# filthyrake/telescope_cam_detection

Hardware: AMD Instinct MI355X
Metric: frames_per_sec (higher is better)
Workload: dtype f16x3; 1 GPU; RT-DETR-R50 640x640 bs=8/GPU, uint8 BGR frames resident in HBM -> [8,300,6] detections in HBM; synthetic seeded weights; global_batch=8, parallelism=camera-shard x1, streams_per_gpu=1, batches_in_flight_per_gpu=1, hip_graph=True

## Files before the change

telescope_cam_detection_amd/csrc/common.h:

```cpp
#pragma once
#include <hip/hip_runtime.h>
#include <stdint.h>
#include <string.h>

#include <stdexcept>
#include <string>
#include <tuple>
#include <type_traits>
#include <utility>
#include <vector>

namespace rtd {

enum DType : int { BF16 = 0, F32 = 1, U8 = 2, I32 = 3, F16X2 = 4 };
constexpr int SPLIT_GROUP = 32;
enum Act : int { ACT_NONE = 0, ACT_RELU = 1, ACT_SILU = 2, ACT_GELU = 3 };
enum ResMode : int { RES_NONE = 0, RES_PRE = 1, RES_POST = 2 };

inline size_t dtype_size(int dt) { return dt == BF16 ? 2 : (dt == U8 ? 1 : 4); }

typedef __bf16 bf16;
typedef __bf16 bf16x8 __attribute__((ext_vector_type(8)));
typedef __bf16 bf16x4 __attribute__((ext_vector_type(4)));
typedef _Float16 sp16;
// ... 125 lines not shown
  const void* pf = nullptr;
  size_t pf_bytes = 0;
};
void launch_conv(const ConvArgs& a, hipStream_t s);
bool conv_dual_supported(const ConvArgs& a);
bool conv_next_supported(const ConvArgs& a);
int conv_kpad(int K);
int conv_kpad_split(int K);
bool conv_split_supported(const ConvArgs& a);
int conv_npad(int N);
bool conv_avg_supported(const ConvArgs& a);
bool conv_sx_batch_fits(const ConvArgs& a);
bool conv_pool_supported(const ConvArgs& a, const Tensor& pooled);
size_t conv_pool_side_bytes(const ConvArgs& a);
void launch_conv_pool(const ConvArgs& a, const Tensor& pooled, void* side, hipStream_t s);
size_t conv_split_slab_bytes(const ConvArgs& a);

void launch_layernorm(const Tensor& x, const Tensor* res, const float* g, const float* b, const Tensor& y,
                      float eps, hipStream_t s);
void launch_add(const Tensor& a, const Tensor& b, const Tensor& y, hipStream_t s);
void launch_maxpool3x3s2(const Tensor& x, const Tensor& y, hipStream_t s);
void launch_upsample2x(const Tensor& x, const Tensor& y, hipStream_t s);
void launch_avgpool2(const Tensor& x, const Tensor& y, hipStream_t s);
void launch_attention(const Tensor& qk, const Tensor& v, const Tensor& o, int heads, hipStream_t s);
void launch_set_rows(const Tensor& y, const int32_t* rows, int nrows, int rows_per_image, const float* vec,
                     hipStream_t s);
void launch_rowmax(const Tensor& x, float* out, hipStream_t s);
void launch_topk(const float* keys, int B, int N, int K, int32_t* idx, float* vals, hipStream_t s);
void launch_gather_rows(const Tensor& src, const int32_t* idx, int rows_per_image, const Tensor& dst, hipStream_t s);
void launch_ref_init(const Tensor& boxdelta, const float* anchors, const int32_t* idx, int S, float* ref_unact8,
// ... 105 lines not shown
__device__ __forceinline__ f32x16 mfma_pair32(const sp16x8& a, const sp16x8& b, const f32x16& c) { return __builtin_amdgcn_mfma_f32_32x32x16_f16(a, b, c, 0, 0, 0); }
__device__ __forceinline__ void split_load8(const sp16* base, long long pix_off, int c, float (&v)[8]) {
  const sp16* q = base + split_off(pix_off, c);
  const sp16x8 h = *(const sp16x8*)q, l = *(const sp16x8*)(q + SPLIT_GROUP);
#pragma unroll
  for (int k = 0; k < 8; ++k) v[k] = (float)h[k] + (float)l[k];
}
__device__ __forceinline__ void split_store8(sp16* base, long long pix_off, int c, const float (&v)[8]) {
  sp16* q = base + split_off(pix_off, c);
  sp16x8 h, l;
#pragma unroll
  for (int k = 0; k < 8; ++k) { sp16 a, b; split2(v[k], a, b); h[k] = a; l[k] = b; }
  *(sp16x8*)q = h;
  *(sp16x8*)(q + SPLIT_GROUP) = l;
}
__device__ __forceinline__ float rows4_max(float v) {
  const auto a = __builtin_amdgcn_permlane16_swap(__float_as_uint(v), __float_as_uint(v), false, false);
  const float t = fmaxf(__uint_as_float(a[0]), __uint_as_float(a[1]));
  const auto b = __builtin_amdgcn_permlane32_swap(__float_as_uint(t), __float_as_uint(t), false, false);
  return fmaxf(__uint_as_float(b[0]), __uint_as_float(b[1]));
}
__device__ __forceinline__ float rows4_sum(float v) {
  const auto a = __builtin_amdgcn_permlane16_swap(__float_as_uint(v), __float_as_uint(v), false, false);
  const float t = __uint_as_float(a[0]) + __uint_as_float(a[1]);
  const auto b = __builtin_amdgcn_permlane32_swap(__float_as_uint(t), __float_as_uint(t), false, false);
  return __uint_as_float(b[0]) + __uint_as_float(b[1]);
}
#define RTD_DPP_ROW_REDUCE(OP)                                                           \
  v = OP(v, __builtin_bit_cast(float, __builtin_amdgcn_update_dpp(0, __builtin_bit_cast(int, v), 0xB1, 0xf, 0xf, false)));   \
  v = OP(v, __builtin_bit_cast(float, __builtin_amdgcn_update_dpp(0, __builtin_bit_cast(int, v), 0x4E, 0xf, 0xf, false)));   \
// ... 23 lines not shown
```

telescope_cam_detection_amd/csrc/conv_igemm.hip:

```cpp
#include <stdlib.h>
#include <string.h>

#include <algorithm>

#include "common.h"

namespace rtd {

struct ConvK {
  const void* x;
  const void* w;
  const float* bias;
  const void* res;
  void* y;
  int M, H, W, Cin;
  long long ldx, x_bstride;
  int OH, OW, OHW;
  int N, Kreal, Kpad;
  int KH, KW, stride, pad;
  long long ldy, y_bstride, ldr, r_bstride;
  int act, res_mode, y_f32, res_f32;
  int ntn;
  const void* pf;
  unsigned pf_bytes;
// ... 1085 lines not shown
  if (four) rtd_launch((conv_igemm_ws_kernel<T, 4>), dim3((unsigned)(mt * ntn)), dim3(512), 0, s, g);
  else rtd_launch((conv_igemm_ws_kernel<T, 2>), dim3((unsigned)(mt * ntn)), dim3(512), 0, s, g);
  return true;
}


struct PoolOut {
  sp16* y;
  long long ldy, bstride;
  int OH, OW;
  unsigned y_bytes;
  sp16* side_row;
  sp16* side_col;
  unsigned row_bytes, col_bytes;
};
template <int COG, bool POOL = false>
__global__ __launch_bounds__(512, 2) void conv3x3_reg_split_kernel(const ConvK a, unsigned x_bytes, unsigned y_bytes, int tiles_x, int tiles_y, int ntiles,
                                                                   const PoolOut po) {
  static_assert(!POOL || COG == 2, "the pooled form is stem.2's (32 -> 64 channels)");
  constexpr int NW = 8, NT_ = 512, WPG = NW / COG, RPW = 8 / WPG;
  constexpr int TH = 8, TW = 32, PW = TW + 2, PH = TH + 2, NPIX = PW * PH;
  constexpr int ROWB = 128, CPP = 8, PPI = 8;
  constexpr int NINSTR = (NPIX + PPI - 1) / PPI;
  constexpr int PBUF = NINSTR * 1024;
  constexpr int ROWO = 128 + 16;
  constexpr int WROW = 9 * 64 * 2 + 16;
  static_assert(32 * COG * WROW <= 2 * PBUF, "the filter is staged through the two patch buffers");
  __shared__ __attribute__((aligned(16))) char patch[2 * PBUF];
  __shared__ __attribute__((aligned(16))) char stage[NW][32 * ROWO];

  const int tid = threadIdx.x, lane = tid & 63;
  const int wv = __builtin_amdgcn_readfirstlane(tid >> 6);
  const int grp = wv / WPG, wq = wv % WPG;
  const int nbase = grp * 32;
  const int h = lane >> 5;

  sp16x8 wf[9][4];
  {
    const sp16* wg = (const sp16*)a.w;
    constexpr int CPR = 9 * 64 / 8;
    for (int e = tid; e < 32 * COG * CPR; e += NT_) {
      const int row = e / CPR, ch = e - row * CPR;
      *(sp16x8*)(patch + row * WROW + ch * 16) = *(const sp16x8*)(wg + (size_t)row * a.Kpad + ch * 8);
    }
    __syncthreads();
#pragma unroll
    for (int tap = 0; tap < 9; ++tap)
#pragma unroll
      for (int kc = 0; kc < 4; ++kc)
        wf[tap][kc] = *(const sp16x8*)(patch + (nbase + (lane & 31)) * WROW + (tap * 64 + kc * 16 + 8 * h) * 2);
    __syncthreads();
  }

  const __amdgpu_buffer_rsrc_t rx = __builtin_amdgcn_make_buffer_rsrc((void*)a.x, 0, x_bytes, 0x00020000);
  const __amdgpu_buffer_rsrc_t ry = __builtin_amdgcn_make_buffer_rsrc(POOL ? (void*)po.y : (void*)a.y, 0, POOL ? po.y_bytes : y_bytes, 0x00020000);
  const __amdgpu_buffer_rsrc_t rsr = __builtin_amdgcn_make_buffer_rsrc((void*)(POOL ? po.side_row : (sp16*)a.y), 0, POOL ? po.row_bytes : 0u, 0x00020000);
  const __amdgpu_buffer_rsrc_t rsc = __builtin_amdgcn_make_buffer_rsrc((void*)(POOL ? po.side_col : (sp16*)a.y), 0, POOL ? po.col_bytes : 0u, 0x00020000);
  auto swz = [](int pi) { return (pi >> 1) & 7; };
  auto issue_patch = [&](int tile, int buf) {
    const int tx = tile % tiles_x;
    const int t2 = tile / tiles_x;
    const int ty = t2 % tiles_y;
    const int b = t2 / tiles_y;
    const int x0 = tx * TW, y0 = ty * TH;
    for (int j = wv; j < NINSTR; j += NW) {
      const int pi = j * PPI + lane / CPP;
      const int py = pi / PW, px = pi - py * PW;
      const int iy = y0 - 1 + py, ix = x0 - 1 + px;
      const bool ok = pi < NPIX && (unsigned)iy < (unsigned)a.H && (unsigned)ix < (unsigned)a.W;
      const int src_chunk = (lane % CPP) ^ swz(pi);
      const unsigned vo = ok ? (unsigned)(((long long)b * a.x_bstride + ((long long)iy * a.W + ix) * a.ldx) * 2 + src_chunk * 16) : 0x80000000u;
      __builtin_amdgcn_raw_ptr_buffer_load_lds(rx, (lds_ptr_t)(patch + buf * PBUF + j * 1024), 16, vo, 0, 0, 0);
    }
  };

  int tile = blockIdx.x;
  if (tile < ntiles) issue_patch(tile, 0);
  for (int it = 0; tile < ntiles; tile += gridDim.x, ++it) {
    const int buf = it & 1;
    if (it == 0) asm volatile("s_waitcnt vmcnt(0)" ::: "memory");
    else if (RPW == 1) asm volatile("s_waitcnt vmcnt(4)" ::: "memory");
    else asm volatile("s_waitcnt vmcnt(8)" ::: "memory");
    __syncthreads();
    if (tile + (int)gridDim.x < ntiles) issue_patch(tile + gridDim.x, buf ^ 1);
    const int tx = tile % tiles_x;
    const int t2 = tile / tiles_x;
    const int ty = t2 % tiles_y;
    const int b = t2 / tiles_y;
    const int x0 = tx * TW, y0 = ty * TH;
    const char* pbuf = patch + buf * PBUF;

    float vm[16];
#pragma unroll
    for (int e = 0; e < 16; ++e) vm[e] = 0.f;
#pragma unroll 1
    for (int rr_ = 0; rr_ < RPW; ++rr_) {
      const int r = wq * RPW + rr_;
      f32x16 acc;
#pragma unroll
      for (int e = 0; e < 16; ++e) acc[e] = 0.f;
      sp16x8 xf[2][4];
      auto read_tap = [&](sp16x8 (&dst)[4], int tap) {
        const int kh = tap / 3, kw = tap - kh * 3;
        const int pi = (r + kh) * PW + kw + (lane & 31);
// ... 794 lines not shown
  k.pf_bytes = (o.prefetch && a.pf && a.pf_bytes < (1ull << 31)) ? (unsigned)a.pf_bytes : 0u;
  const long long x_bytes = ((long long)(x.n - 1) * x.bstride + ((long long)x.h * x.w - 1) * x.ld + x.c) * 4;
  const long long w_bytes = (long long)a.Npad * a.Kpad * 2;
  RTD_CHECK(x_bytes < (1ll << 31) && x2_bytes < (1ll << 31) && w_bytes < (1ll << 31), 1, "conv (f16x3): operand larger than a buffer descriptor (2 GiB)");
  g.splitk = 1; g.x_bytes = (unsigned)x_bytes; g.w_bytes = (unsigned)w_bytes; g.x2_bytes = (unsigned)x2_bytes;
  if (dispatch_sx(k, a, x_bytes, x2_bytes, s)) { HIP_CHECK(hipGetLastError()); return; }
  RTD_CHECK(a.next_y.p == nullptr, 1, "conv (f16x3): a fused following conv exists in the streaming kernel only");
  RTD_CHECK(a.avg_y.p == nullptr, 1, "conv (f16x3): the fused vd-shortcut average exists in the streaming kernel only (the plan must fall back to the avg-pool launch)");
  if (o.conv_reg && a.KH == 3 && a.KW == 3 && a.stride == 1 && a.pad == 1 && !dual && a.res_mode == RES_NONE && x.c == 32 && (y.c == 32 || y.c == 64) &&
      y.dt == F16X2) {
    const long long y_bytes = ((long long)(y.n - 1) * y.bstride + ((long long)y.h * y.w - 1) * y.ld + y.c) * 4;
    const int tiles_x = (x.w + 31) / 32, tiles_y = (x.h + 7) / 8;
    const long long ntiles = (long long)x.n * tiles_x * tiles_y;
    if (tiles_x * tiles_y >= 32 && ntiles < (1ll << 30) && y_bytes < (1ll << 31)) {
      const unsigned gx = (unsigned)std::min<long long>(ntiles, 256);
      if (y.c == 32) rtd_launch((conv3x3_reg_split_kernel<1>), dim3(gx), dim3(512), 0, s, k, (unsigned)x_bytes, (unsigned)y_bytes, tiles_x, tiles_y, (int)ntiles, PoolOut{});
      else rtd_launch((conv3x3_reg_split_kernel<2>), dim3(gx), dim3(512), 0, s, k, (unsigned)x_bytes, (unsigned)y_bytes, tiles_x, tiles_y, (int)ntiles, PoolOut{});
      HIP_CHECK(hipGetLastError());
      return;
    }
  }
  if ((o.conv_reg & 2) && a.KH == 3 && a.KW == 3 && a.stride == 1 && a.pad == 1 && !dual && a.res_mode == RES_NONE && x.c == 64 && y.c == 64 && y.dt == F16X2) {
    const long long y_bytes = ((long long)(y.n - 1) * y.bstride + ((long long)y.h * y.w - 1) * y.ld + y.c) * 4;
    const int tiles_x = (x.w + 15) / 16, tiles_y = (x.h + 7) / 8;
    const long long ntiles = (long long)x.n * tiles_x * tiles_y;
    if (tiles_x * tiles_y >= 128 && ntiles < (1ll << 30) && y_bytes < (1ll << 31)) {
      const unsigned gx = (unsigned)std::min<long long>(ntiles, 256);
      rtd_launch(conv3x3_reg_split64_kernel, dim3(gx), dim3(512), 0, s, k, (unsigned)x_bytes, (unsigned)y_bytes, tiles_x, tiles_y, (int)ntiles);
      HIP_CHECK(hipGetLastError());
      return;
    }
  }
// ... 117 lines not shown
  k.KH = 3; k.KW = 3; k.stride = 1; k.pad = 1;
  k.ldy = 0; k.y_bstride = 0; k.ldr = 0; k.r_bstride = 0; k.res_f32 = 0;
  k.act = a.act; k.res_mode = RES_NONE; k.y_f32 = 0; k.split = 1; k.y_split = 1; k.res_split = 0;
  k.x2 = nullptr; k.ldx2 = 0; k.x2_bstride = 0; k.k2_start = 0; k.ntn = 1; k.reg_epi = 1; k.prefer256 = 0; k.pf = nullptr; k.pf_bytes = 0; k.x_up2 = 0;
  k.next_w = nullptr; k.next_bias = nullptr; k.next_y = nullptr; k.next_ldy = 0; k.next_y_bstride = 0; k.next_kpad = 0; k.next_act = 0;
  const long long x_bytes = ((long long)(x.n - 1) * x.bstride + ((long long)x.h * x.w - 1) * x.ld + x.c) * 4;
  const long long p_bytes = ((long long)(pooled.n - 1) * pooled.bstride + ((long long)pooled.h * pooled.w - 1) * pooled.ld + pooled.c) * 4;
  const int tiles_x = (x.w + 31) / 32, tiles_y = (x.h + 7) / 8;
  const long long ntiles = (long long)x.n * tiles_x * tiles_y;
  RTD_CHECK(x_bytes < (1ll << 31) && p_bytes < (1ll << 31) && ntiles * 8192 < (1ll << 31), 1, "conv + max-pool: operand larger than a buffer descriptor");
  PoolOut po;
  po.y = (sp16*)pooled.p; po.ldy = pooled.ld; po.bstride = pooled.bstride; po.OH = pooled.h; po.OW = pooled.w; po.y_bytes = (unsigned)p_bytes;
  po.side_row = (sp16*)side; po.row_bytes = (unsigned)(ntiles * 8192);
  po.side_col = (sp16*)((char*)side + ntiles * 8192); po.col_bytes = (unsigned)(ntiles * 1024);
  const unsigned gx = (unsigned)std::min<long long>(ntiles, 256);
  rtd_launch((conv3x3_reg_split_kernel<2, true>), dim3(gx), dim3(512), 0, s, k, (unsigned)x_bytes, 0u, tiles_x, tiles_y, (int)ntiles, po);
  HIP_CHECK(hipGetLastError());
  const long long items = ntiles * 19 * (64 / 8);
  rtd_launch(k_pool_fixup, dim3((unsigned)((items + 255) / 256)), dim3(256), 0, s, po, tiles_x, tiles_y, (int)ntiles, 64);
  HIP_CHECK(hipGetLastError());
}

void launch_conv(const ConvArgs& a, hipStream_t s) {
  const Tensor& x = a.x;
  const Tensor& y = a.y;
  if (x.dt == F16X2) { launch_conv_split(a, s); return; }
  const ConvOpts& o = opts_of(a);
  RTD_CHECK(x.dt == BF16 || x.dt == F32, 1, "conv: input dtype");
  RTD_CHECK(y.dt == BF16 || y.dt == F32 || (y.dt == F16X2 && x.dt == F32), 1, "conv: output dtype");
  if (y.dt == F16X2) RTD_CHECK(y.c % SPLIT_GROUP == 0 && y.ld % SPLIT_GROUP == 0 && a.res_mode == RES_NONE && !a.x2.p && !a.next_y.p && ((uintptr_t)y.p & 15) == 0, 1,
                                "conv: fp32 -> F16X2 output needs 32-channel groups and no residual / second input");
  const int epc = x.dt == BF16 ? 8 : 4;
  const int up = a.x_up2 ? 2 : 1;
  if (a.x_up2) RTD_CHECK(a.KH == 1 && a.KW == 1 && a.stride == 1 && a.pad == 0 && a.x2.p, 1, "conv: x_up2 needs a 1x1 conv with a second input");
// ... 73 lines not shown
```

telescope_cam_detection_amd/csrc/engine.hip:

```cpp
#include "engine_internal.h"

using namespace rtd;
using namespace rtd_eng;

namespace rtd {
__thread GraphBuild* t_graph_build = nullptr;
__thread long long t_launches = 0;
}

void launch_force_idx(int32_t* dst, const int32_t* src, const int32_t* flag, int n, hipStream_t s);

namespace rtd_eng {
thread_local std::string g_create_error;
PlanOpts g_opts;
}

namespace rtd_eng {

void parse_blob(rtd_engine* e) {
  const char* b = e->blob.data();
  const size_t n = e->blob.size();
  RTD_CHECK(n >= 12 && memcmp(b, "RTDW", 4) == 0, RTD_E_WEIGHTS, "weight blob: bad magic");
  uint32_t ver, count;
  memcpy(&ver, b + 4, 4);
// ... 479 lines not shown
  Tensor encoder(Flow& F);
  bool dec_fused() const { return e->opts.dec_fused && c.d_model == 256 && c.dec_heads == 8 && c.dec_ffn <= 1024 && c.num_classes <= 512 && c.n_levels == 3 && c.n_points == 4; }
  Queries select_queries(Flow& F, const Tensor& mem);
  Decoded decoder(Flow& F, const Tensor& mem, const Queries& q);
  Tensor decoder_fused(Flow& F, const Queries& q, const Tensor& vall, float* ref8, float* ref_unact8);
  Tensor decoder_by_op(const Queries& q, const Tensor& vall, const Tensor& ref8t, float* ref_unact8);
  void post_process(const Decoded& d);
};

void Builder::stem(Flow& F) {
  const int H = c.input_h, W = c.input_w;
  Tensor x = act(SP ? F32 : P, n, H, W, 8, "input");
  plan->input = x;
  const int eh = c.embedding_size / 2;
  const int h = down2(H), w = down2(W);
  Tensor s0 = act(P, n, h, w, eh);
  plan->stem_fused = SP && e->opts.stem_fused_split && eh == 32;
  if (plan->stem_fused) {
    const uint8_t** table = (const uint8_t**)alloc((size_t)c.max_batch * sizeof(void*));
    plan->frame_table = table;
    if (!dry) {
      DevWeight w0 = get_weight(e, {{"backbone.stem.0", 9 * 8}}, P, eh);
      const void* wp = w0.w; const float* bp = w0.bias; const int kp = w0.Kpad; const int n = this->n;
      push("backbone.stem.0", "conv_igemm", 2.0 * n * h * w * eh * 27.0, (double)n * H * W * 3 + tbytes(s0),
           [table, n, H, W, wp, kp, bp, s0](hipStream_t st) { launch_stem0_u8(table, n, H, W, wp, kp, bp, s0, ACT_RELU, st); });
    }
  } else {
    conv("backbone.stem.0", x, s0, {.k = 3, .stride = 2, .pad = 1, .act = ACT_RELU, .real_cin = 3});
  }
  Tensor s1 = act(P, n, h, w, eh);
  conv("backbone.stem.1", s0, s1, {.k = 3, .pad = 1, .act = ACT_RELU});
  const Tensor s2v = mk(nullptr, P, n, h, w, c.embedding_size);
  const int ph = down2(h), pw = down2(w);
  const ConvSpec stem2{.k = 3, .pad = 1, .act = ACT_RELU};
  const long long pool_tiles = (long long)n * ((w + 31) / 32) * ((h + 7) / 8);
  const bool fuse = SP && e->opts.stem_pool_fuse && conv_pool_supported(probe(s1, s2v, stem2), probe_shape(mk(nullptr, P, n, ph, pw, c.embedding_size), 1)) &&
                    pool_tiles * 8192 < (1ll << 31);
  F.h = ph; F.w = pw;
  if (fuse) {
    F.cur = act(P, n, ph, pw, c.embedding_size, "stem");
    ConvArgs a;
    a.x = s1; a.y = s2v;
    a.KH = a.KW = 3; a.stride = 1; a.pad = 1; a.act = ACT_RELU; a.opts = &e->conv_opts;
    const DevWeight w2 = get_weight(e, {{"backbone.stem.2", 9 * s1.c}}, P, c.embedding_size, dry);
    a.w = w2.w; a.bias = w2.bias; a.Kpad = w2.Kpad; a.Npad = w2.Npad;
    void* side = alloc(conv_pool_side_bytes(a));
// ... 1105 lines not shown
```

telescope_cam_detection_amd/csrc/engine_internal.h:

```cpp
#pragma once
#include <math.h>
#include <string.h>

#include <chrono>
#include <functional>
#include <map>
#include <memory>
#include <mutex>
#include <string>
#include <vector>

#include "../../include/rtdetr_mi355.h"
#include "../../include/rtdetr_mi355_test.h"
#include "common.h"

namespace rtd_eng {
using namespace rtd;

struct PlanOpts {
  int sc_fold = 1;
  int c1_fuse = 1;
  int attn_split = 3;
  int up_fold = 1;
  int arena_reuse = 1;
  int stem_fused_split = 1;
  int aifi_pair = 1;
  int post_fused = 1;
  int dead_out = 1;
  int avg_fuse = 1;
  int stem_pool_fuse = 1;
  int sel_fused = 1;
  int dec_fused = 1;
  int side_stream = 7;
};

struct HostTensor {
  const float* data = nullptr;
  std::vector<int64_t> shape;
  int64_t numel() const {
    int64_t n = 1;
    for (auto d : shape) n *= d;
    return n;
  }
};
// ... 144 lines not shown
```

telescope_cam_detection_amd/csrc/ops.hip:

```cpp
#include <float.h>

#include <algorithm>

#include "common.h"

namespace rtd {

template <typename T> __device__ __forceinline__ float ldf(const T* p) { return (float)(*p); }
template <typename T> __device__ __forceinline__ void stf(T* p, float v) { *p = (T)v; }

__device__ __forceinline__ float wave_sum(float v) { return wave_sum64(v); }

static inline unsigned blocks_for(int64_t n, int per_block) { return (unsigned)((n + per_block - 1) / per_block); }

#define DISPATCH_T(dt, ...)                     \
  do {                                          \
    if ((dt) == BF16) { typedef bf16 T; __VA_ARGS__; } \
    else { typedef float T; __VA_ARGS__; }      \
  } while (0)

template <typename T>
__global__ void k_f32_to(const float* __restrict__ src, T* __restrict__ dst, int64_t n) {
  int64_t i = (int64_t)blockIdx.x * blockDim.x + threadIdx.x;
  if (i < n) dst[i] = (T)src[i];
// ... 1289 lines not shown
  __shared__ __attribute__((aligned(16))) char stage[4][32 * ROWO];
  const int tid = threadIdx.x, lane = tid & 63, wv = tid >> 6, h = lane >> 5;
  int t = blockIdx.x;
  const int tx = t % tiles_x; t /= tiles_x;
  const int ty = t % tiles_y;
  const int b = t / tiles_y;
  const int x0 = tx * TW, y0 = ty * TH;
  const uint8_t* __restrict__ f = table[b];
  const long long fbytes = (long long)H * W * 3;
  const bool aligned4 = (((uintptr_t)f) & 3) == 0;
  for (int e = tid; e < PR * NDW; e += 256) {
    const int r = e / NDW, d = e - r * NDW;
    const int iy = 2 * y0 - 1 + r;
    const long long g0 = ((long long)iy * W + (2 * x0 - 1)) * 3;
    const long long a0 = (g0 & ~3ll) + 4ll * d;
    unsigned dw = 0;
    const bool row_ok = (unsigned)iy < (unsigned)H;
    if (row_ok) {
      if (aligned4 && a0 >= 0 && a0 + 4 <= fbytes) dw = *(const unsigned*)(f + a0);
      else {
#pragma unroll
        for (int q = 0; q < 4; ++q)
          if (a0 + q >= 0 && a0 + q < fbytes) dw |= (unsigned)f[a0 + q] << (8 * q);
      }
    }
#pragma unroll
    for (int q = 0; q < 4; ++q) {
      const int el = (int)(a0 + q - g0);
      if (el < 0 || el >= PC * 3) continue;
      const int ix = 2 * x0 - 1 + el / 3;
      const float v = (row_ok && (unsigned)ix < (unsigned)W) ? (float)((dw >> (8 * q)) & 0xffu) : 0.f;
      const float vn = v / 255.0f;
      const E hi = (E)vn;
      patch[r * ROWE + el] = hi;
      if (SPLIT) patch_lo[r * ROWE + el] = (E)(vn - (float)hi);
    }
  }
  for (int e = tid; e < PR * (ROWE - PC * 3); e += 256) {
    const int r = e / (ROWE - PC * 3), i = e - r * (ROWE - PC * 3);
    patch[r * ROWE + PC * 3 + i] = (E)0.f;
    if (SPLIT) patch_lo[r * ROWE + PC * 3 + i] = (E)0.f;
  }
  Ex8 wf[2], wfl[2];
  int doff[2][4];
#pragma unroll
  for (int s = 0; s < 2; ++s) {
#pragma unroll
    for (int j = 0; j < 8; ++j) {
      const int k = 16 * s + 8 * h + j;
      const int kh = k / 10, e = k - kh * 10;
      const int kw = e / 3, cb = e - kw * 3;
      const int kr = (kh * 3 + kw) * 8 + (2 - cb);
      const bool real = k < 30 && e < 9;
      if (SPLIT) {
        const size_t pos = (size_t)(lane & 31) * Kpad + ((kr >> 5) << 6) + (kr & 31);
        wf[s][j] = real ? wq[pos] : (E)0.f;
        wfl[s][j] = real ? wq[pos + 32] : (E)0.f;
      } else {
        wf[s][j] = real ? wq[(size_t)(lane & 31) * Kpad + kr] : (E)0.f;
      }
    }
#pragma unroll
    for (int j = 0; j < 4; ++j) {
      const int k = 16 * s + 8 * h + 2 * j;
      const int kh = k / 10, e = k - kh * 10;
      doff[s][j] = k < 30 ? kh * ROWE + e : 0;
    }
  }
  __syncthreads();
#pragma unroll 1
  for (int rr = 0; rr < 2; ++rr) {
    const int r = wv * 2 + rr;
    const int eoff = (2 * r) * ROWE + (2 * (lane & 31)) * 3;
    const E* base = patch + eoff;
    f32x16_s acc;
#pragma unroll
    for (int e = 0; e < 16; ++e) acc[e] = 0.f;
#pragma unroll
    for (int s = 0; s < 2; ++s) {
      typedef unsigned u4_s __attribute__((ext_vector_type(4)));
      unsigned xd[4];
#pragma unroll
      for (int j = 0; j < 4; ++j) xd[j] = *(const unsigned*)(base + doff[s][j]);
      const u4_s xv = {xd[0], xd[1], xd[2], xd[3]};
      if constexpr (SPLIT) acc = mfma_pair32(wf[s], __builtin_bit_cast(Ex8, xv), acc);
      else acc = __builtin_amdgcn_mfma_f32_32x32x16_bf16(wf[s], __builtin_bit_cast(Ex8, xv), acc, 0, 0, 0);
      if constexpr (SPLIT) {
        unsigned xl[4];
#pragma unroll
        for (int j = 0; j < 4; ++j) xl[j] = *(const unsigned*)(patch_lo + eoff + doff[s][j]);
        const u4_s xlv = {xl[0], xl[1], xl[2], xl[3]};
        acc = mfma_pair32(wf[s], __builtin_bit_cast(Ex8, xlv), acc);
        acc = mfma_pair32(wfl[s], __builtin_bit_cast(Ex8, xv), acc);
      }
    }
    const int oy = y0 + r;
    char* sw_ = stage[wv];
#pragma unroll
    for (int q = 0; q < 4; ++q) {
      const f32x4_s bv = *(const f32x4_s*)(bias + 8 * q + 4 * h);
      Ex4 o, ol;
#pragma unroll
      for (int e = 0; e < 4; ++e) {
        float v = acc[4 * q + e] + bv[e];
        if (act == ACT_RELU) v = fmaxf(v, 0.f);
        else if (act == ACT_SILU) v = v / (1.f + __expf(-v));
        if constexpr (SPLIT) { sp16 hh, ll; split2(v, hh, ll); o[e] = hh; ol[e] = ll; }
        else o[e] = (E)v;
      }
      *(Ex4*)(sw_ + (lane & 31) * ROWO + (8 * q + 4 * h) * 2) = o;
// ... 69 lines not shown
```

telescope_cam_detection_amd/csrc/testapi.hip:

```cpp
#include "engine_internal.h"

using namespace rtd;
using namespace rtd_eng;

extern "C" {

int rtd_debug_tensor(rtd_handle h, const char* name, float* out, int64_t capacity, int64_t shape[4]) {
  return guarded(h, [&] {
    RTD_CHECK(name && shape && h->last_n > 0, RTD_E_STATE, "no forward has run");
    Plan* p = h->plans[h->last_n].get();
    auto it = p->named.find(name);
    RTD_CHECK(it != p->named.end(), RTD_E_INVALID, std::string("unknown debug tensor ") + name);
    const Tensor& t = it->second;
    if (p->stem_fused && strcmp(name, "input") == 0 && out) {
      HIP_CHECK(hipSetDevice(h->cfg.device));
      launch_preprocess_identity(h->last_fa, h->cfg.input_h, h->cfg.input_w, p->input, p->scale_wh, h->stream);
    }
    shape[0] = t.n; shape[1] = t.h; shape[2] = t.w; shape[3] = t.c;
    const int64_t numel = t.pixels() * t.c;
    if (!out) return;
    RTD_CHECK(capacity >= numel, RTD_E_INVALID, "debug tensor: output capacity too small");
    RTD_CHECK(t.bstride == (int64_t)t.h * t.w * t.ld, RTD_E_INVALID, "debug tensor: non-dense batch stride");
    HIP_CHECK(hipSetDevice(h->cfg.device));
    const size_t es = dtype_size(t.dt);
// ... 147 lines not shown
  for (int i = 0; i < 16; ++i) s += acc[i][0] + acc[i][3];
  if (s == 123.456f) sink[0] = s;
  if (lane == 0) { const int w = blockIdx.x * 4 + (tid >> 6); out[2 * w] = c1 - c0; out[2 * w + 1] = r1 - r0; }
}
static int g_bench_rewarm = 0;
int rtd_debug_option(const char* name, int value) {
  if (!name) return RTD_E_INVALID;
  if (strcmp(name, "reset") == 0) {
    g_opts = PlanOpts();
    g_profile_twice = 0; g_bench_rewarm = 0;
    conv_opts_template() = ConvOpts();
    return RTD_OK;
  }
  const struct { const char* n; int* p; } plan_opts[] = {
      {"dec_fused", &g_opts.dec_fused}, {"side_stream", &g_opts.side_stream}, {"sel_fused", &g_opts.sel_fused},
      {"stem_fused_split", &g_opts.stem_fused_split}, {"stem_pool_fuse", &g_opts.stem_pool_fuse}, {"avg_fuse", &g_opts.avg_fuse}, {"dead_out", &g_opts.dead_out}, {"post_fused", &g_opts.post_fused}, {"aifi_pair", &g_opts.aifi_pair}, {"sc_fold", &g_opts.sc_fold}, {"arena_reuse", &g_opts.arena_reuse},
      {"up_fold", &g_opts.up_fold}, {"attn_split", &g_opts.attn_split}, {"c1_fuse", &g_opts.c1_fuse},
      {"profile_twice", &g_profile_twice}, {"bench_rewarm", &g_bench_rewarm},
  };
  for (const auto& t : plan_opts)
    if (strcmp(name, t.n) == 0) { *t.p = value; return RTD_OK; }
  if (conv_set_option(name, value)) return RTD_OK;
  return RTD_E_INVALID;
}

struct DevFilter {
  float* wpad = nullptr; void* w = nullptr; float* bias = nullptr;
  int Kpad = 0, Npad = 0;
  void release() { if (w != wpad) (void)hipFree(w); (void)hipFree(wpad); (void)hipFree(bias); }
};
static DevFilter dev_filter(int dtype, const void* w_f32, const float* bias, int N, int K) {
// ... 302 lines not shown
```

Measured before the change: 1838 frames/s.

## Fuse stem.0 uint8 conv into stem.1 conv kernel via on-chip recompute

```diff
diff --git a/telescope_cam_detection_amd/csrc/common.h b/telescope_cam_detection_amd/csrc/common.h
--- a/telescope_cam_detection_amd/csrc/common.h
+++ b/telescope_cam_detection_amd/csrc/common.h
@@ -163,6 +163,10 @@
 bool conv_pool_supported(const ConvArgs& a, const Tensor& pooled);
 size_t conv_pool_side_bytes(const ConvArgs& a);
 void launch_conv_pool(const ConvArgs& a, const Tensor& pooled, void* side, hipStream_t s);
+bool stem01_u8_supported(const ConvArgs& a);
+bool stem01_u8_batch_fits(const ConvArgs& a);
+void launch_stem01_u8(const uint8_t* const* table_dev, int n, int H, int W, const void* w0, int Kpad0, const float* bias0, const ConvArgs& a,
+                      hipStream_t s);
 size_t conv_split_slab_bytes(const ConvArgs& a);
 
 void launch_layernorm(const Tensor& x, const Tensor* res, const float* g, const float* b, const Tensor& y,
@@ -298,6 +302,81 @@
   *(sp16x8*)q = h;
   *(sp16x8*)(q + SPLIT_GROUP) = l;
 }
+__device__ __forceinline__ unsigned stem_u8_fetch(const uint8_t* __restrict__ f, long long fbytes, bool aligned4, bool row_ok, long long a0) {
+  unsigned dw = 0;
+  if (row_ok) {
+    if (aligned4 && a0 >= 0 && a0 + 4 <= fbytes) dw = *(const unsigned*)(f + a0);
+    else {
+#pragma unroll
+      for (int q = 0; q < 4; ++q)
+        if (a0 + q >= 0 && a0 + q < fbytes) dw |= (unsigned)f[a0 + q] << (8 * q);
+    }
+  }
+  return dw;
+}
+__device__ __forceinline__ void stem_u8_put(unsigned dw, long long a0, long long g0, bool row_ok, int xbase, int W, int nel, sp16* __restrict__ hi_row,
+                                            sp16* __restrict__ lo_row) {
+#pragma unroll
+  for (int q = 0; q < 4; ++q) {
+    const int el = (int)(a0 + q - g0);
+    if (el < 0 || el >= nel) continue;
+    const int ix = xbase + el / 3;
+    const float v = (row_ok && (unsigned)ix < (unsigned)W) ? (float)((dw >> (8 * q)) & 0xffu) : 0.f;
+    const float vn = v / 255.0f;
+    const sp16 hi = (sp16)vn;
+    hi_row[el] = hi;
+    lo_row[el] = (sp16)(vn - (float)hi);
+  }
+}
+struct Stem0Frags {
+  sp16x8 wh[2], wl[2];
+  int doff[2][4];
+};
+__device__ __forceinline__ Stem0Frags stem0_u8_frags(const sp16* __restrict__ wq, int Kpad, int lane, int rowe) {
+  Stem0Frags fr;
+  const int h = lane >> 5;
+#pragma unroll
+  for (int s = 0; s < 2; ++s) {
+#pragma unroll
+    for (int j = 0; j < 8; ++j) {
+      const int k = 16 * s + 8 * h + j;
+      const int kh = k / 10, e = k - kh * 10;
+      const int kw = e / 3, cb = e - kw * 3;
+      const int kr = (kh * 3 + kw) * 8 + (2 - cb);
+      const bool real = k < 30 && e < 9;
+      const size_t pos = (size_t)(lane & 31) * Kpad + ((kr >> 5) << 6) + (kr & 31);
+      fr.wh[s][j] = real ? wq[pos] : (sp16)0.f;
+      fr.wl[s][j] = real ? wq[pos + 32] : (sp16)0.f;
+    }
+#pragma unroll
+    for (int j = 0; j < 4; ++j) {
+      const int k = 16 * s + 8 * h + 2 * j;
+      const int kh = k / 10, e = k - kh * 10;
+      fr.doff[s][j] = k < 30 ? kh * rowe + e : 0;
+    }
+  }
+  return fr;
+}
+__device__ __forceinline__ f32x16 stem0_u8_mfma(const Stem0Frags& fr, const sp16* hi, const sp16* lo) {
+  typedef unsigned u4_s __attribute__((ext_vector_type(4)));
+  f32x16 acc;
+#pragma unroll
+  for (int e = 0; e < 16; ++e) acc[e] = 0.f;
+#pragma unroll
+  for (int s = 0; s < 2; ++s) {
+    unsigned xd[4], xl[4];
+#pragma unroll
+    for (int j = 0; j < 4; ++j) xd[j] = *(const unsigned*)(hi + fr.doff[s][j]);
+    const u4_s xv = {xd[0], xd[1], xd[2], xd[3]};
+    acc = mfma_pair32(fr.wh[s], __builtin_bit_cast(sp16x8, xv), acc);
+#pragma unroll
+    for (int j = 0; j < 4; ++j) xl[j] = *(const unsigned*)(lo + fr.doff[s][j]);
+    const u4_s xlv = {xl[0], xl[1], xl[2], xl[3]};
+    acc = mfma_pair32(fr.wh[s], __builtin_bit_cast(sp16x8, xlv), acc);
+    acc = mfma_pair32(fr.wl[s], __builtin_bit_cast(sp16x8, xv), acc);
+  }
+  return acc;
+}
 __device__ __forceinline__ float rows4_max(float v) {
   const auto a = __builtin_amdgcn_permlane16_swap(__float_as_uint(v), __float_as_uint(v), false, false);
   const float t = fmaxf(__uint_as_float(a[0]), __uint_as_float(a[1]));
diff --git a/telescope_cam_detection_amd/csrc/conv_igemm.hip b/telescope_cam_detection_amd/csrc/conv_igemm.hip
--- a/telescope_cam_detection_amd/csrc/conv_igemm.hip
+++ b/telescope_cam_detection_amd/csrc/conv_igemm.hip
@@ -1123,10 +1123,18 @@
   sp16* side_col;
   unsigned row_bytes, col_bytes;
 };
-template <int COG, bool POOL = false>
+struct Stem0In {
+  const uint8_t* const* table;
+  int H, W;
+  const sp16* w;
+  int Kpad;
+  const float* bias;
+};
+template <int COG, bool POOL = false, bool U8 = false>
 __global__ __launch_bounds__(512, 2) void conv3x3_reg_split_kernel(const ConvK a, unsigned x_bytes, unsigned y_bytes, int tiles_x, int tiles_y, int ntiles,
-                                                                   const PoolOut po) {
+                                                                   const PoolOut po, const Stem0In s0) {
   static_assert(!POOL || COG == 2, "the pooled form is stem.2's (32 -> 64 channels)");
+  static_assert(!U8 || (COG == 1 && !POOL), "the uint8 form is stem.1's (32 -> 32 channels)");
   constexpr int NW = 8, NT_ = 512, WPG = NW / COG, RPW = 8 / WPG;
   constexpr int TH = 8, TW = 32, PW = TW + 2, PH = TH + 2, NPIX = PW * PH;
   constexpr int ROWB = 128, CPP = 8, PPI = 8;
@@ -1134,9 +1142,22 @@
   constexpr int PBUF = NINSTR * 1024;
   constexpr int ROWO = 128 + 16;
   constexpr int WROW = 9 * 64 * 2 + 16;
-  static_assert(32 * COG * WROW <= 2 * PBUF, "the filter is staged through the two patch buffers");
-  __shared__ __attribute__((aligned(16))) char patch[2 * PBUF];
+  constexpr int NBUF = U8 ? 1 : 2;
+  static_assert(U8 || 32 * COG * WROW <= NBUF * PBUF, "the filter is staged through the patch buffers");
+  __shared__ __attribute__((aligned(16))) char patch_s[NBUF * PBUF];
   __shared__ __attribute__((aligned(16))) char stage[NW][32 * ROWO];
+  constexpr int UR = 2 * PH + 1, UC = 2 * PW + 1, UROW = 212, UNDW = (UC * 3 + 3 + 3) / 4, UPT = (UR * UNDW + NT_ - 1) / NT_;
+  static_assert(UROW % 2 == 0 && UROW >= 6 * (PW - 1) + 10, "a pixel's 10-element filter row stays inside its patch row");
+  __shared__ __attribute__((aligned(16))) sp16 u8hi_s[U8 ? UR * UROW : 8];
+  __shared__ __attribute__((aligned(16))) sp16 u8lo_s[U8 ? UR * UROW : 8];
+  __shared__ __attribute__((aligned(16))) Stem0Frags fr0_s[U8 ? 64 : 1];
+  Stem0Frags* const fr0p = fr0_s;
+  constexpr int RELOAD = 2;
+  __shared__ __attribute__((aligned(16))) char wlds_s[U8 ? 32 * WROW : 16];
+  char* const wbuf = U8 ? wlds_s : patch_s;
+  char* const patch = patch_s;
+  sp16* const u8hi = u8hi_s;
+  sp16* const u8lo = u8lo_s;
 
   const int tid = threadIdx.x, lane = tid & 63;
   const int wv = __builtin_amdgcn_readfirstlane(tid >> 6);
@@ -1150,14 +1171,14 @@
     constexpr int CPR = 9 * 64 / 8;
     for (int e = tid; e < 32 * COG * CPR; e += NT_) {
       const int row = e / CPR, ch = e - row * CPR;
-      *(sp16x8*)(patch + row * WROW + ch * 16) = *(const sp16x8*)(wg + (size_t)row * a.Kpad + ch * 8);
+      *(sp16x8*)(wbuf + row * WROW + ch * 16) = *(const sp16x8*)(wg + (size_t)row * a.Kpad + ch * 8);
     }
     __syncthreads();
 #pragma unroll
     for (int tap = 0; tap < 9; ++tap)
 #pragma unroll
       for (int kc = 0; kc < 4; ++kc)
-        wf[tap][kc] = *(const sp16x8*)(patch + (nbase + (lane & 31)) * WROW + (tap * 64 + kc * 16 + 8 * h) * 2);
+        wf[tap][kc] = *(const sp16x8*)(wbuf + (nbase + (lane & 31)) * WROW + (tap * 64 + kc * 16 + 8 * h) * 2);
     __syncthreads();
   }
 
@@ -1183,20 +1204,98 @@
     }
   };
 
+  const long long fbytes = (long long)s0.H * s0.W * 3;
+  auto u8_item = [&](int tile, int i, const uint8_t*& f, int& r, long long& g0, long long& a0, bool& row_ok, int& xbase) {
+    const int tx = tile % tiles_x;
+    const int t2 = tile / tiles_x;
+    const int ty = t2 % tiles_y;
+    f = s0.table[t2 / tiles_y];
+    const int e = tid + i * NT_;
+    r = e / UNDW;
+    const int iy = 2 * (ty * TH) - 3 + r;
+    xbase = 2 * (tx * TW) - 3;
+    g0 = ((long long)iy * s0.W + xbase) * 3;
+    a0 = (g0 & ~3ll) + 4ll * (e - r * UNDW);
+    row_ok = (unsigned)iy < (unsigned)s0.H;
+    return e < UR * UNDW;
+  };
+  auto u8_fetch = [&](int tile, unsigned (&dw)[UPT]) {
+#pragma unroll
+    for (int i = 0; i < UPT; ++i) {
+      const uint8_t* f; int r, xbase; long long g0, a0; bool row_ok;
+      dw[i] = u8_item(tile, i, f, r, g0, a0, row_ok, xbase) ? stem_u8_fetch(f, fbytes, (((uintptr_t)f) & 3) == 0, row_ok, a0) : 0u;
+    }
+  };
+  auto u8_put = [&](int tile, const unsigned (&dw)[UPT]) {
+#pragma unroll
+    for (int i = 0; i < UPT; ++i) {
+      const uint8_t* f; int r, xbase; long long g0, a0; bool row_ok;
+      if (u8_item(tile, i, f, r, g0, a0, row_ok, xbase)) stem_u8_put(dw[i], a0, g0, row_ok, xbase, s0.W, UC * 3, u8hi + r * UROW, u8lo + r * UROW);
+    }
+  };
+  unsigned udw[UPT];
+
   int tile = blockIdx.x;
-  if (tile < ntiles) issue_patch(tile, 0);
+  if constexpr (U8) {
+    if (tile < ntiles) u8_fetch(tile, udw);
+    if (wv == 0) fr0p[lane] = stem0_u8_frags(s0.w, s0.Kpad, lane, UROW);
+    for (int e = tid; e < UR * (UROW - UC * 3); e += NT_) {
+      const int r = e / (UROW - UC * 3), i = e - r * (UROW - UC * 3);
+      u8hi[r * UROW + UC * 3 + i] = (sp16)0.f;
+      u8lo[r * UROW + UC * 3 + i] = (sp16)0.f;
+    }
+  } else {
+    if (tile < ntiles) issue_patch(tile, 0);
+  }
   for (int it = 0; tile < ntiles; tile += gridDim.x, ++it) {
-    const int buf = it & 1;
-    if (it == 0) asm volatile("s_waitcnt vmcnt(0)" ::: "memory");
-    else if (RPW == 1) asm volatile("s_waitcnt vmcnt(4)" ::: "memory");
-    else asm volatile("s_waitcnt vmcnt(8)" ::: "memory");
-    __syncthreads();
-    if (tile + (int)gridDim.x < ntiles) issue_patch(tile + gridDim.x, buf ^ 1);
+    const int buf = U8 ? 0 : (it & 1);
     const int tx = tile % tiles_x;
     const int t2 = tile / tiles_x;
     const int ty = t2 % tiles_y;
     const int b = t2 / tiles_y;
     const int x0 = tx * TW, y0 = ty * TH;
+    if constexpr (U8) {
+      u8_put(tile, udw);
+      __syncthreads();
+      if (tile + (int)gridDim.x < ntiles) u8_fetch(tile + gridDim.x, udw);
+      const Stem0Frags fr0 = fr0p[lane];
+      for (int g = wv; g * 32 < NPIX; g += NW) {
+        const int pi = g * 32 + (lane & 31), pic = pi < NPIX ? pi : NPIX - 1;
+        const int py = pic / PW, px = pic - py * PW;
+        const int eoff = 2 * py * UROW + 6 * px;
+        const f32x16 acc = stem0_u8_mfma(fr0, u8hi + eoff, u8lo + eoff);
+        const bool in_map = (unsigned)(y0 - 1 + py) < (unsigned)a.H && (unsigned)(x0 - 1 + px) < (unsigned)a.W;
+        char* prow = patch + pic * ROWB;
+        const int sw = swz(pic);
+#pragma unroll
+        for (int q = 0; q < 4; ++q) {
+          const f32x4 bv = *(const f32x4*)(s0.bias + 8 * q + 4 * h);
+          sp16x4 oh, ol;
+#pragma unroll
+          for (int e = 0; e < 4; ++e) {
+            sp16 hi, lo;
+            split2(in_map ? fmaxf(acc[4 * q + e] + bv[e], 0.f) : 0.f, hi, lo);
+            oh[e] = hi; ol[e] = lo;
+          }
+          if (pi < NPIX) {
+            *(sp16x4*)(prow + ((q ^ sw) << 4) + 8 * h) = oh;
+            *(sp16x4*)(prow + (((4 + q) ^ sw) << 4) + 8 * h) = ol;
+          }
+        }
+      }
+      __syncthreads();
+#pragma unroll
+      for (int tap = 9 - RELOAD; tap < 9; ++tap)
+#pragma unroll
+        for (int kc = 0; kc < 4; ++kc)
+          wf[tap][kc] = *(const sp16x8*)(wbuf + (nbase + (lane & 31)) * WROW + (tap * 64 + kc * 16 + 8 * h) * 2);
+    } else {
+      if (it == 0) asm volatile("s_waitcnt vmcnt(0)" ::: "memory");
+      else if (RPW == 1) asm volatile("s_waitcnt vmcnt(4)" ::: "memory");
+      else asm volatile("s_waitcnt vmcnt(8)" ::: "memory");
+      __syncthreads();
+      if (tile + (int)gridDim.x < ntiles) issue_patch(tile + gridDim.x, buf ^ 1);
+    }
     const char* pbuf = patch + buf * PBUF;
 
     float vm[16];
@@ -2021,8 +2120,8 @@
     const long long ntiles = (long long)x.n * tiles_x * tiles_y;
     if (tiles_x * tiles_y >= 32 && ntiles < (1ll << 30) && y_bytes < (1ll << 31)) {
       const unsigned gx = (unsigned)std::min<long long>(ntiles, 256);
-      if (y.c == 32) rtd_launch((conv3x3_reg_split_kernel<1>), dim3(gx), dim3(512), 0, s, k, (unsigned)x_bytes, (unsigned)y_bytes, tiles_x, tiles_y, (int)ntiles, PoolOut{});
-      else rtd_launch((conv3x3_reg_split_kernel<2>), dim3(gx), dim3(512), 0, s, k, (unsigned)x_bytes, (unsigned)y_bytes, tiles_x, tiles_y, (int)ntiles, PoolOut{});
+      if (y.c == 32) rtd_launch((conv3x3_reg_split_kernel<1>), dim3(gx), dim3(512), 0, s, k, (unsigned)x_bytes, (unsigned)y_bytes, tiles_x, tiles_y, (int)ntiles, PoolOut{}, Stem0In{});
+      else rtd_launch((conv3x3_reg_split_kernel<2>), dim3(gx), dim3(512), 0, s, k, (unsigned)x_bytes, (unsigned)y_bytes, tiles_x, tiles_y, (int)ntiles, PoolOut{}, Stem0In{});
       HIP_CHECK(hipGetLastError());
       return;
     }
@@ -2170,10 +2269,51 @@
   po.side_row = (sp16*)side; po.row_bytes = (unsigned)(ntiles * 8192);
   po.side_col = (sp16*)((char*)side + ntiles * 8192); po.col_bytes = (unsigned)(ntiles * 1024);
   const unsigned gx = (unsigned)std::min<long long>(ntiles, 256);
-  rtd_launch((conv3x3_reg_split_kernel<2, true>), dim3(gx), dim3(512), 0, s, k, (unsigned)x_bytes, 0u, tiles_x, tiles_y, (int)ntiles, po);
+  rtd_launch((conv3x3_reg_split_kernel<2, true>), dim3(gx), dim3(512), 0, s, k, (unsigned)x_bytes, 0u, tiles_x, tiles_y, (int)ntiles, po, Stem0In{});
   HIP_CHECK(hipGetLastError());
   const long long items = ntiles * 19 * (64 / 8);
   rtd_launch(k_pool_fixup, dim3((unsigned)((items + 255) / 256)), dim3(256), 0, s, po, tiles_x, tiles_y, (int)ntiles, 64);
+  HIP_CHECK(hipGetLastError());
+}
+
+bool stem01_u8_supported(const ConvArgs& a) {
+  const Tensor& x = a.x;
+  const Tensor& y = a.y;
+  if (x.dt != F16X2 || y.dt != F16X2 || x.c != 32 || y.c != 32 || y.h != x.h || y.w != x.w || y.ld % SPLIT_GROUP) return false;
+  if (!(a.KH == 3 && a.KW == 3 && a.stride == 1 && a.pad == 1 && !a.x2.p && !a.next_y.p && !a.avg_y.p && a.res_mode == RES_NONE && a.act == ACT_RELU)) return false;
+  if (((uintptr_t)y.p & 15) || ((uintptr_t)a.w & 15)) return false;
+  const int tiles_x = (x.w + 31) / 32, tiles_y = (x.h + 7) / 8;
+  return tiles_x * tiles_y >= 32 && opts_of(a).conv_reg != 0;
+}
+bool stem01_u8_batch_fits(const ConvArgs& a) {
+  const Tensor& y = a.y;
+  const long long y_bytes = ((long long)(y.n - 1) * y.bstride + ((long long)y.h * y.w - 1) * y.ld + y.c) * 4;
+  const long long ntiles = (long long)y.n * ((y.w + 31) / 32) * ((y.h + 7) / 8);
+  return ntiles < (1ll << 30) && y_bytes < (1ll << 31);
+}
+void launch_stem01_u8(const uint8_t* const* table_dev, int n, int H, int W, const void* w0, int Kpad0, const float* bias0, const ConvArgs& a,
+                      hipStream_t s) {
+  const Tensor& y = a.y;
+  RTD_CHECK(stem01_u8_supported(a) && stem01_u8_batch_fits(a) && table_dev && w0 && bias0 && y.n >= n && n >= 1 && y.h == (H - 1) / 2 + 1 &&
+                y.w == (W - 1) / 2 + 1, 1, "stem.0 + stem.1: shape not supported");
+  ConvK k;
+  k.x = nullptr; k.w = a.w; k.bias = a.bias; k.y = y.p; k.res = nullptr;
+  k.H = y.h; k.W = y.w; k.M = n * y.h * y.w;
+  k.Cin = 64; k.ldx = 0; k.x_bstride = 0;
+  k.OH = y.h; k.OW = y.w; k.OHW = y.h * y.w;
+  k.N = 32; k.Kreal = 2 * 9 * 32; k.Kpad = a.Kpad;
+  k.KH = 3; k.KW = 3; k.stride = 1; k.pad = 1;
+  k.ldy = y.ld; k.y_bstride = y.bstride; k.ldr = 0; k.r_bstride = 0; k.res_f32 = 0;
+  k.act = a.act; k.res_mode = RES_NONE; k.y_f32 = 0; k.split = 1; k.y_split = 1; k.res_split = 0;
+  k.x2 = nullptr; k.ldx2 = 0; k.x2_bstride = 0; k.k2_start = 0; k.ntn = 1; k.reg_epi = 1; k.prefer256 = 0; k.pf = nullptr; k.pf_bytes = 0; k.x_up2 = 0;
+  k.next_w = nullptr; k.next_bias = nullptr; k.next_y = nullptr; k.next_ldy = 0; k.next_y_bstride = 0; k.next_kpad = 0; k.next_act = 0;
+  const long long y_bytes = ((long long)(n - 1) * y.bstride + ((long long)y.h * y.w - 1) * y.ld + y.c) * 4;
+  const int tiles_x = (y.w + 31) / 32, tiles_y = (y.h + 7) / 8;
+  const long long ntiles = (long long)n * tiles_x * tiles_y;
+  Stem0In s0;
+  s0.table = table_dev; s0.H = H; s0.W = W; s0.w = (const sp16*)w0; s0.Kpad = Kpad0; s0.bias = bias0;
+  const unsigned gx = (unsigned)std::min<long long>(ntiles, 256);
+  rtd_launch((conv3x3_reg_split_kernel<1, false, true>), dim3(gx), dim3(512), 0, s, k, 0u, (unsigned)y_bytes, tiles_x, tiles_y, (int)ntiles, PoolOut{}, s0);
   HIP_CHECK(hipGetLastError());
 }
 
diff --git a/telescope_cam_detection_amd/csrc/engine.hip b/telescope_cam_detection_amd/csrc/engine.hip
--- a/telescope_cam_detection_amd/csrc/engine.hip
+++ b/telescope_cam_detection_amd/csrc/engine.hip
@@ -517,22 +517,40 @@
   plan->input = x;
   const int eh = c.embedding_size / 2;
   const int h = down2(H), w = down2(W);
-  Tensor s0 = act(P, n, h, w, eh);
   plan->stem_fused = SP && e->opts.stem_fused_split && eh == 32;
+  const Tensor s0v = mk(nullptr, P, n, h, w, eh), s1v = mk(nullptr, P, n, h, w, eh);
+  const ConvSpec stem1{.k = 3, .pad = 1, .act = ACT_RELU};
+  const bool fuse01 = plan->stem_fused && e->opts.stem01_fuse && stem01_u8_supported(probe(s0v, s1v, stem1)) && stem01_u8_batch_fits(probe(s0v, s1v, stem1, true));
+  Tensor s0 = fuse01 ? s0v : act(P, n, h, w, eh);
+  Tensor s1;
   if (plan->stem_fused) {
     const uint8_t** table = (const uint8_t**)alloc((size_t)c.max_batch * sizeof(void*));
     plan->frame_table = table;
-    if (!dry) {
+    const int n = this->n;
+    if (fuse01) {
+      s1 = act(P, n, h, w, eh, "stem1");
+      const DevWeight w0 = get_weight(e, {{"backbone.stem.0", 9 * 8}}, P, eh, dry);
+      const DevWeight w1 = get_weight(e, {{"backbone.stem.1", 9 * eh}}, P, eh, dry);
+      ConvArgs a;
+      a.x = s0v; a.y = s1;
+      a.KH = a.KW = 3; a.stride = 1; a.pad = 1; a.act = ACT_RELU; a.opts = &e->conv_opts;
+      a.w = w1.w; a.bias = w1.bias; a.Kpad = w1.Kpad; a.Npad = w1.Npad;
+      const void* wp = w0.w; const float* bp = w0.bias; const int kp = w0.Kpad;
+      push("backbone.stem.0+1", "conv_igemm", 2.0 * n * h * w * eh * 27.0 + 2.0 * n * h * w * eh * 9.0 * eh, (double)n * H * W * 3 + tbytes(s1),
+           [table, n, H, W, wp, kp, bp, a](hipStream_t st) { launch_stem01_u8(table, n, H, W, wp, kp, bp, a, st); });
+    } else if (!dry) {
       DevWeight w0 = get_weight(e, {{"backbone.stem.0", 9 * 8}}, P, eh);
-      const void* wp = w0.w; const float* bp = w0.bias; const int kp = w0.Kpad; const int n = this->n;
+      const void* wp = w0.w; const float* bp = w0.bias; const int kp = w0.Kpad;
       push("backbone.stem.0", "conv_igemm", 2.0 * n * h * w * eh * 27.0, (double)n * H * W * 3 + tbytes(s0),
            [table, n, H, W, wp, kp, bp, s0](hipStream_t st) { launch_stem0_u8(table, n, H, W, wp, kp, bp, s0, ACT_RELU, st); });
     }
   } else {
     conv("backbone.stem.0", x, s0, {.k = 3, .stride = 2, .pad = 1, .act = ACT_RELU, .real_cin = 3});
   }
-  Tensor s1 = act(P, n, h, w, eh);
-  conv("backbone.stem.1", s0, s1, {.k = 3, .pad = 1, .act = ACT_RELU});
+  if (!fuse01) {
+    s1 = act(P, n, h, w, eh, "stem1");
+    conv("backbone.stem.1", s0, s1, stem1);
+  }
   const Tensor s2v = mk(nullptr, P, n, h, w, c.embedding_size);
   const int ph = down2(h), pw = down2(w);
   const ConvSpec stem2{.k = 3, .pad = 1, .act = ACT_RELU};
diff --git a/telescope_cam_detection_amd/csrc/engine_internal.h b/telescope_cam_detection_amd/csrc/engine_internal.h
--- a/telescope_cam_detection_amd/csrc/engine_internal.h
+++ b/telescope_cam_detection_amd/csrc/engine_internal.h
@@ -28,6 +28,7 @@
   int post_fused = 1;
   int dead_out = 1;
   int avg_fuse = 1;
+  int stem01_fuse = 1;
   int stem_pool_fuse = 1;
   int sel_fused = 1;
   int dec_fused = 1;
diff --git a/telescope_cam_detection_amd/csrc/ops.hip b/telescope_cam_detection_amd/csrc/ops.hip
--- a/telescope_cam_detection_amd/csrc/ops.hip
+++ b/telescope_cam_detection_amd/csrc/ops.hip
@@ -1327,86 +1327,22 @@
     const int iy = 2 * y0 - 1 + r;
     const long long g0 = ((long long)iy * W + (2 * x0 - 1)) * 3;
     const long long a0 = (g0 & ~3ll) + 4ll * d;
-    unsigned dw = 0;
     const bool row_ok = (unsigned)iy < (unsigned)H;
-    if (row_ok) {
-      if (aligned4 && a0 >= 0 && a0 + 4 <= fbytes) dw = *(const unsigned*)(f + a0);
-      else {
-#pragma unroll
-        for (int q = 0; q < 4; ++q)
-          if (a0 + q >= 0 && a0 + q < fbytes) dw |= (unsigned)f[a0 + q] << (8 * q);
-      }
-    }
-#pragma unroll
-    for (int q = 0; q < 4; ++q) {
-      const int el = (int)(a0 + q - g0);
-      if (el < 0 || el >= PC * 3) continue;
-      const int ix = 2 * x0 - 1 + el / 3;
-      const float v = (row_ok && (unsigned)ix < (unsigned)W) ? (float)((dw >> (8 * q)) & 0xffu) : 0.f;
-      const float vn = v / 255.0f;
-      const E hi = (E)vn;
-      patch[r * ROWE + el] = hi;
-      if (SPLIT) patch_lo[r * ROWE + el] = (E)(vn - (float)hi);
-    }
+    const unsigned dw = stem_u8_fetch(f, fbytes, aligned4, row_ok, a0);
+    stem_u8_put(dw, a0, g0, row_ok, 2 * x0 - 1, W, PC * 3, patch + r * ROWE, patch_lo + r * ROWE);
   }
   for (int e = tid; e < PR * (ROWE - PC * 3); e += 256) {
     const int r = e / (ROWE - PC * 3), i = e - r * (ROWE - PC * 3);
     patch[r * ROWE + PC * 3 + i] = (E)0.f;
     if (SPLIT) patch_lo[r * ROWE + PC * 3 + i] = (E)0.f;
   }
-  Ex8 wf[2], wfl[2];
-  int doff[2][4];
-#pragma unroll
-  for (int s = 0; s < 2; ++s) {
-#pragma unroll
-    for (int j = 0; j < 8; ++j) {
-      const int k = 16 * s + 8 * h + j;
-      const int kh = k / 10, e = k - kh * 10;
-      const int kw = e / 3, cb = e - kw * 3;
-      const int kr = (kh * 3 + kw) * 8 + (2 - cb);
-      const bool real = k < 30 && e < 9;
-      if (SPLIT) {
-        const size_t pos = (size_t)(lane & 31) * Kpad + ((kr >> 5) << 6) + (kr & 31);
-        wf[s][j] = real ? wq[pos] : (E)0.f;
-        wfl[s][j] = real ? wq[pos + 32] : (E)0.f;
-      } else {
-        wf[s][j] = real ? wq[(size_t)(lane & 31) * Kpad + kr] : (E)0.f;
-      }
-    }
-#pragma unroll
-    for (int j = 0; j < 4; ++j) {
-      const int k = 16 * s + 8 * h + 2 * j;
-      const int kh = k / 10, e = k - kh * 10;
-      doff[s][j] = k < 30 ? kh * ROWE + e : 0;
-    }
-  }
+  const Stem0Frags fr = stem0_u8_frags(wq, Kpad, lane, ROWE);
   __syncthreads();
 #pragma unroll 1
   for (int rr = 0; rr < 2; ++rr) {
     const int r = wv * 2 + rr;
     const int eoff = (2 * r) * ROWE + (2 * (lane & 31)) * 3;
-    const E* base = patch + eoff;
-    f32x16_s acc;
-#pragma unroll
-    for (int e = 0; e < 16; ++e) acc[e] = 0.f;
-#pragma unroll
-    for (int s = 0; s < 2; ++s) {
-      typedef unsigned u4_s __attribute__((ext_vector_type(4)));
-      unsigned xd[4];
-#pragma unroll
-      for (int j = 0; j < 4; ++j) xd[j] = *(const unsigned*)(base + doff[s][j]);
-      const u4_s xv = {xd[0], xd[1], xd[2], xd[3]};
-      if constexpr (SPLIT) acc = mfma_pair32(wf[s], __builtin_bit_cast(Ex8, xv), acc);
-      else acc = __builtin_amdgcn_mfma_f32_32x32x16_bf16(wf[s], __builtin_bit_cast(Ex8, xv), acc, 0, 0, 0);
-      if constexpr (SPLIT) {
-        unsigned xl[4];
-#pragma unroll
-        for (int j = 0; j < 4; ++j) xl[j] = *(const unsigned*)(patch_lo + eoff + doff[s][j]);
-        const u4_s xlv = {xl[0], xl[1], xl[2], xl[3]};
-        acc = mfma_pair32(wf[s], __builtin_bit_cast(Ex8, xlv), acc);
-        acc = mfma_pair32(wfl[s], __builtin_bit_cast(Ex8, xv), acc);
-      }
-    }
+    const f32x16 acc = stem0_u8_mfma(fr, patch + eoff, patch_lo + eoff);
     const int oy = y0 + r;
     char* sw_ = stage[wv];
 #pragma unroll
diff --git a/telescope_cam_detection_amd/csrc/testapi.hip b/telescope_cam_detection_amd/csrc/testapi.hip
--- a/telescope_cam_detection_amd/csrc/testapi.hip
+++ b/telescope_cam_detection_amd/csrc/testapi.hip
@@ -185,7 +185,7 @@
   }
   const struct { const char* n; int* p; } plan_opts[] = {
       {"dec_fused", &g_opts.dec_fused}, {"side_stream", &g_opts.side_stream}, {"sel_fused", &g_opts.sel_fused},
-      {"stem_fused_split", &g_opts.stem_fused_split}, {"stem_pool_fuse", &g_opts.stem_pool_fuse}, {"avg_fuse", &g_opts.avg_fuse}, {"dead_out", &g_opts.dead_out}, {"post_fused", &g_opts.post_fused}, {"aifi_pair", &g_opts.aifi_pair}, {"sc_fold", &g_opts.sc_fold}, {"arena_reuse", &g_opts.arena_reuse},
+      {"stem_fused_split", &g_opts.stem_fused_split}, {"stem01_fuse", &g_opts.stem01_fuse}, {"stem_pool_fuse", &g_opts.stem_pool_fuse}, {"avg_fuse", &g_opts.avg_fuse}, {"dead_out", &g_opts.dead_out}, {"post_fused", &g_opts.post_fused}, {"aifi_pair", &g_opts.aifi_pair}, {"sc_fold", &g_opts.sc_fold}, {"arena_reuse", &g_opts.arena_reuse},
       {"up_fold", &g_opts.up_fold}, {"attn_split", &g_opts.attn_split}, {"c1_fuse", &g_opts.c1_fuse},
       {"profile_twice", &g_profile_twice}, {"bench_rewarm", &g_bench_rewarm},
   };
```

After: 1845 frames/s, median of 6. No clear change (+0.4%).
